# bioinfo-pf-curie/mpiBWA

Hardware: AMD Instinct MI355X
Metric: Mreads/s (whole node) 2x150 bp PE vs GRCh38-size reference; SAM bit-match (higher is better)
Workload: dtype int32

## Files before the change

### include/mpibwa_amd.h

```cpp
#ifndef MPIBWA_AMD_H
#define MPIBWA_AMD_H

#include <stdint.h>
#include <stddef.h>
#include <stdio.h>

#ifdef __cplusplus
extern "C" {
#endif

#define MEM_F_PE             0x2
#define MEM_F_NOPAIRING      0x4
#define MEM_F_ALL            0x8
#define MEM_F_NO_MULTI       0x10
#define MEM_F_NO_RESCUE      0x20
#define MEM_F_REF_HDR        0x100
#define MEM_F_SOFTCLIP       0x200
#define MEM_F_SMARTPE        0x400
#define MEM_F_PRIMARY5       0x800
#define MEM_F_KEEP_SUPP_MAPQ 0x1000

typedef uint64_t bwtint_t;

typedef struct {
// ... 132 lines not shown
int mi355x_smem_batch(const mem_opt_t *opt, int n, const uint8_t *seqs, const int64_t *off,
                      int cap, uint64_t *intv_out, int *n_out, double *kernel_ms, uint64_t *algo_bytes);
int mi355x_sa_batch(int n, const uint64_t *k, uint64_t *sa_out, double *kernel_ms, uint64_t *algo_bytes);
int mi355x_sa_batch2(int n, const uint64_t *k, uint64_t *sa_out, double *kernel_ms, int dense);
double mi355x_sa_dense_info(size_t *bytes);
int mi355x_extend_batch(const mem_opt_t *opt, int n, const uint8_t *q, const int64_t *qoff,
                        const uint8_t *t, const int64_t *toff, const int *w, const int *h0,
                        const int *end_bonus, int *out6, double *kernel_ms, uint64_t *cells);
int mi355x_extend_batch2(const mem_opt_t *opt, int n, const uint8_t *q, const int64_t *qoff,
                         const uint8_t *t, const int64_t *toff, const int *w, const int *h0,
                         const int *end_bonus, const int *early, const int *clip, int *out6,
                         uint64_t *cells, double *kernel_ms);

int64_t mi355x_chain_batch(const mem_opt_t *opt, const bntseq_t *bns, int n_reads, const int *lens, const int *l_rep,
                           const int64_t *seed_off, const uint64_t *rbeg, const int32_t *qbeg_len, int which,
                           int64_t *out, int64_t out_cap, int64_t *out_off);

int64_t mi355x_c2a_batch(const mem_opt_t *opt, const bntseq_t *bns, int n_reads, const uint8_t *reads, const int64_t *off,
                         const int *n_chains, const int *chain_rid, const float *chain_frac, const int *chain_nseeds,
                         const int64_t *seed_rbeg, const int *seed_qbeg, const int *seed_len, const int *seed_score,
                         int heavy_t, int early, int layout, int64_t *out, int64_t out_cap, int64_t *out_off,
                         uint64_t *stat4, int *n_units);

int mi355x_global_batch(const mem_opt_t *opt, int64_t l_pac, const uint8_t *pac, int n_reads, const uint8_t *reads,
                        const int64_t *off, int n_req, const int64_t *rb, const int64_t *re, const int *read,
                        const int *qb, const int *qe, const int *w, const int *truesc, int which,
                        int *out_hdr5, uint32_t *cigar_out, int cigar_cap, char *md_out, int md_cap, double *kernel_ms);
void mi355x_global_batch_counts(uint64_t out[4]);

int mi355x_pair_maxreg(void);
int mi355x_pair_batch(const mem_opt_t *opt, const bntseq_t *bns, const mem_pestat_t pes[4], int64_t n_processed, int n_pairs,
                      const void *regs, const int *n_regs, int max_len, uint8_t *status, void *desc, void *req);

int mi355x_pair_wave_maxreg(void);
int mi355x_pair_wave_batch(const mem_opt_t *opt, const bntseq_t *bns, const uint8_t *pac, const mem_pestat_t pes[4], int64_t n_processed,
                           int n_pairs, const uint8_t *reads, const int64_t *off, const void *regs, const int *reg_off, uint8_t *status,
                           void *desc, void *req, int *n_align);

int mi355x_pair_wave_xa_cap(void);
int mi355x_pair_wave_xa_batch(const mem_opt_t *opt, const bntseq_t *bns, const uint8_t *pac, const mem_pestat_t pes[4], int64_t n_processed,
                              int n_pairs, const uint8_t *reads, const int64_t *off, const void *regs, const int *reg_off, uint8_t *status,
                              void *desc, void *req, int *n_align, void *xa_req, uint8_t *xa_cnt);

int mi355x_pair_wave_lines_batch(const mem_opt_t *opt, const bntseq_t *bns, const uint8_t *pac, const mem_pestat_t pes[4], int64_t n_processed,
                                 int n_pairs, const uint8_t *reads, const int64_t *off, const void *regs, const int *reg_off, uint8_t *status,
                                 void *desc, void *req, int *n_align, void *xa_req, uint8_t *xa_cnt, uint8_t *n_lines, void *line_desc,
// ... 118 lines not shown
```

### mpibwa_amd/api.py

```python
import ctypes as C
import os

import numpy as np

from . import abi

HERE = os.path.dirname(os.path.abspath(__file__))
_LIB = None

libc = C.CDLL(None if os.environ.get("MPIBWA_SANITIZER_LIB") else "libc.so.6")
libc.free.argtypes = [C.c_void_p]

EXPORTS = [
    "mem_process_seqs", "mem_opt_init", "bwa_fill_scmat", "bwa_idx_load_from_disk", "bwa_mem2idx", "bwa_idx_destroy",
    "mi355x_index_upload", "mi355x_index_alloc", "mi355x_index_buffers", "mi355x_index_d2d", "mi355x_index_commit",
    "mi355x_finalize", "mi355x_index_build", "mi355x_index_build_gpu",
    "mi355x_smem_batch", "mi355x_sa_batch", "mi355x_sa_batch2", "mi355x_sa_dense_info", "mi355x_extend_batch", "mi355x_extend_batch2", "mi355x_matesw_batch", "mi355x_matesw_batch_counts", "mi355x_chain_batch", "mi355x_c2a_batch", "mi355x_pair_batch", "mi355x_pair_maxreg", "mi355x_fastq_scan", "mi355x_fastq_chunks", "mi355x_fastq_fill", "mi355x_last_stats", "mi355x_host_cpus", "mi355x_collect_sam", "mi355x_collect_sam_into", "mi355x_host_ksw_align2",
    "bwa_set_rg", "bwa_insert_header", "bwa_idx2mem", "mi355x_write_map", "mi355x_init", "mi355x_rank_host_threads", "mi355x_index_checksums", "mi355x_init_bcast_seconds", "mi355x_global_batch", "mi355x_global_batch_counts", "mi355x_device_count", "mi355x_device_cus", "mi355x_device_memory", "mi355x_buffer_growths", "mi355x_prewarm", "mi355x_max_calls",
    "mi355x_sam_batch", "mi355x_sam_arena_bytes", "mi355x_se_batch", "mi355x_sam_se_batch", "mi355x_seed_batch", "mi355x_pair_wave_batch", "mi355x_pair_wave_maxreg",
    "mi355x_pair_wave_xa_batch", "mi355x_pair_wave_xa_cap", "mi355x_dedup_batch", "mi355x_dedup_maxreg", "mi355x_se_wave_batch",
    "mi355x_se_lines_cap", "mi355x_se_wave_lines_batch", "mi355x_sam_se_lines_batch", "mi355x_sam_lines_row", "mi355x_sam_lines_sa_stage",
    "mi355x_pair_wave_lines_batch", "mi355x_sam_pe_lines_batch",
]


class mi355x_comm_t(C.Structure):
    BCAST = C.CFUNCTYPE(None, C.c_void_p, C.c_size_t, C.c_int, C.c_void_p)
    _fields_ = [("rank", C.c_int), ("size", C.c_int), ("bcast", BCAST), ("user", C.c_void_p)]



def load_library(build_if_missing=True):
    global _LIB
    if _LIB is not None:
        return _LIB
    path = os.path.join(HERE, "libmpibwa_amd.so")
    host_only = os.environ.get("MPIBWA_SANITIZER_LIB")
    if host_only:
        path = host_only
    if not os.path.exists(path):
        if not build_if_missing or host_only:
            raise RuntimeError("%s is missing: run python -m mpibwa_amd.build" % path)
        from .build import build
        build()
    lib = C.CDLL(path)
# ... 10 lines not shown
        fn.argtypes = argtypes

    sig("mem_opt_init", P(abi.mem_opt_t), [])
    sig("bwa_idx_load_from_disk", P(abi.bwaidx_t), [C.c_char_p, C.c_int])
    sig("mi355x_index_build", C.c_int, [C.c_char_p, C.c_char_p])
    sig("mi355x_index_build_gpu", C.c_int, [C.c_int, C.c_void_p, C.c_int64, C.c_char_p, P(C.c_double)])
    sig("mem_process_seqs", None, [P(abi.mem_opt_t), P(abi.bwt_t), P(abi.bntseq_t), P(C.c_uint8), C.c_int64, C.c_int,
                                   P(abi.bseq1_t), P(abi.mem_pestat_t)])
    sig("mi355x_index_upload", C.c_int, [C.c_int, P(abi.bwt_t), P(abi.bntseq_t), P(C.c_uint8)])
    sig("mi355x_index_alloc", C.c_int, [C.c_int, P(abi.bwt_t), P(abi.bntseq_t)])
    sig("mi355x_index_buffers", C.c_int, [P(C.c_void_p), P(C.c_size_t)] * 3)
    sig("mi355x_index_d2d", C.c_int, [C.c_int, C.c_void_p, C.c_size_t, C.c_int])
    sig("mi355x_index_commit", C.c_int, [])
    sig("mi355x_smem_batch", C.c_int, [P(abi.mem_opt_t), C.c_int, C.c_void_p, C.c_void_p, C.c_int, C.c_void_p,
                                       C.c_void_p, P(C.c_double), P(C.c_uint64)])
    sig("mi355x_sa_batch", C.c_int, [C.c_int, C.c_void_p, C.c_void_p, P(C.c_double), P(C.c_uint64)])
    sig("mi355x_sa_batch2", C.c_int, [C.c_int, C.c_void_p, C.c_void_p, P(C.c_double), C.c_int])
    sig("mi355x_sa_dense_info", C.c_double, [P(C.c_size_t)])
    sig("mi355x_extend_batch", C.c_int, [P(abi.mem_opt_t), C.c_int] + [C.c_void_p] * 8 + [P(C.c_double), P(C.c_uint64)])
    sig("mi355x_extend_batch2", C.c_int, [P(abi.mem_opt_t), C.c_int] + [C.c_void_p] * 11 + [P(C.c_double)])
    sig("mi355x_chain_batch", C.c_int64, [P(abi.mem_opt_t), C.c_void_p, C.c_int] + [C.c_void_p] * 5 + [C.c_int, C.c_void_p, C.c_int64, C.c_void_p])
    sig("mi355x_c2a_batch", C.c_int64, [P(abi.mem_opt_t), C.c_void_p, C.c_int] + [C.c_void_p] * 10 + [C.c_int] * 3 +
        [C.c_void_p, C.c_int64, C.c_void_p, C.c_void_p, C.c_void_p])
    sig("mi355x_fastq_scan", C.c_int64, [C.c_void_p, C.c_int64, C.c_int64, C.c_void_p, C.c_void_p])
    sig("mi355x_fastq_chunks", C.c_int64, [C.c_void_p, C.c_void_p, C.c_int64, C.c_int64, C.c_int64, C.c_void_p])
    sig("mi355x_fastq_fill", C.c_int64, [C.c_void_p, C.c_void_p, C.c_void_p, C.c_void_p, C.c_int64, C.c_int64, C.c_int, C.c_int, C.c_void_p])
    sig("mi355x_matesw_batch", C.c_int, [P(abi.mem_opt_t), C.c_int64, C.c_void_p, C.c_int, C.c_void_p, C.c_void_p, C.c_int] + [C.c_void_p] * 5 + [P(C.c_double)])
    sig("mi355x_last_stats", None, [P(abi.mi355x_stats_t)])
    sig("mi355x_finalize", None, [])
    sig("mi355x_host_ksw_align2", None, [C.c_int, C.c_void_p, C.c_int, C.c_void_p, C.c_void_p] + [C.c_int] * 6 + [C.c_void_p])
    sig("mi355x_host_cpus", C.c_int, [])
    sig("mi355x_host_sort_dedup_patch", C.c_int, [P(abi.mem_opt_t), P(abi.bntseq_t), C.c_void_p, C.c_void_p, C.c_void_p, C.c_int])
    sig("mi355x_host_reg2sam_se", None, [P(abi.mem_opt_t), P(abi.bntseq_t), C.c_void_p, P(abi.bseq1_t), C.c_void_p, C.c_int, C.c_int64])
    sig("mi355x_host_pestat", None, [P(abi.mem_opt_t), C.c_int64, C.c_int, C.c_void_p, C.c_void_p, C.c_void_p, C.c_int])
    sig("mi355x_host_flt_chained_seeds", None, [P(abi.mem_opt_t), P(abi.bntseq_t), C.c_void_p, C.c_int, C.c_void_p, C.c_int, C.c_void_p, C.c_void_p])
    sig("mi355x_host_sam_pe", C.c_int, [P(abi.mem_opt_t), P(abi.bntseq_t), C.c_void_p, C.c_void_p, C.c_uint64, P(abi.bseq1_t), C.c_void_p, C.c_int, C.c_void_p, C.c_int])
    sig("mi355x_collect_sam", C.c_void_p, [P(abi.bseq1_t), C.c_int, P(C.c_size_t)])
    sig("mi355x_fixmate_pair", C.c_int, [P(abi.bseq1_t), P(abi.bseq1_t), P(abi.bntseq_t)])
    sig("mi355x_fixmate", C.c_int64, [P(abi.bseq1_t), C.c_int, P(abi.bntseq_t)])
    sig("mi355x_bgzf_bound", C.c_size_t, [C.c_size_t])
    sig("mi355x_bgzf_compress", C.c_size_t, [C.c_char_p, C.c_size_t, C.c_int, C.c_void_p, C.c_size_t])
    sig("mi355x_bgzf_eof", C.c_size_t, [C.c_void_p])
    sig("mi355x_bgzf_compress_dev", C.c_size_t, [C.c_char_p, C.c_size_t, C.c_void_p, C.c_size_t])
    sig("mi355x_bgzf_dev_counts", None, [P(C.c_uint64)])
    sig("mi355x_bgzf_find_block", C.c_int64, [C.c_char_p, C.c_int64, C.c_int])
    sig("mi355x_bgzf_scan", C.c_int64, [C.c_char_p, C.c_int64, C.c_int64, P(C.c_int64), P(C.c_int64)])
# ... 242 lines not shown
        rid = np.array([c[0] for c in ch] or [0], dtype=np.int32)
        frac = np.array([c[1] for c in ch] or [0], dtype=np.float32)
        nsd = np.array([len(c[2]) for c in ch] or [0], dtype=np.int32)
        sd = np.array([s for c in ch for s in c[2]] or [(0, 0, 0, 0)], dtype=np.int64).reshape(-1, 4)
        rbeg = np.ascontiguousarray(sd[:, 0])
        qbeg, ln, sc = (np.ascontiguousarray(sd[:, k], dtype=np.int32) for k in (1, 2, 3))
        cap = n + 11 * max(int(nsd.sum()), 1) + 64
        out = np.zeros(cap, dtype=np.int64)
        out_off = np.zeros(n + 1, dtype=np.int64)
        stat = np.zeros(4, dtype=np.uint64)
        units = C.c_int(0)
        rc = self.lib.mi355x_c2a_batch(opt, C.cast(self.bns, C.c_void_p), n, flat.ctypes.data, off.ctypes.data, n_chains.ctypes.data, rid.ctypes.data,
                                       frac.ctypes.data, nsd.ctypes.data, rbeg.ctypes.data, qbeg.ctypes.data, ln.ctypes.data, sc.ctypes.data,
                                       int(heavy_t), int(early), int(layout), out.ctypes.data, cap, out_off.ctypes.data, stat.ctypes.data, C.addressof(units))
        assert rc >= 0
        res = []
        for r in range(n):
            p = int(out_off[r])
            m = int(out[p])
            res.append(out[p + 1:p + 1 + 11 * m].reshape(m, 11).copy())
        st = dict(zip(("cells", "n_ext", "n_closed", "n_diff"), (int(x) for x in stat)))
        return res, st, units.value

    REG_DT = np.dtype([("rb", "<i8"), ("re", "<i8"), ("qb", "<i4"), ("qe", "<i4"), ("rid", "<i4"), ("score", "<i4"), ("truesc", "<i4"), ("w", "<i4"),
                       ("seedcov", "<i4"), ("seedlen0", "<i4"), ("frac_rep", "<f4"), ("pad", "<i4")])
    DESC_DT = np.dtype([("rb", "<i8"), ("re", "<i8"), ("qb", "<i4"), ("qe", "<i4"), ("req", "<i4"), ("rid", "<i4"), ("flag", "<i4"), ("mapq", "<i4"),
                        ("score", "<i4"), ("sub", "<i4")])
    AREQ_DT = np.dtype([("rb", "<i8"), ("re", "<i8"), ("read", "<i4"), ("qb", "<i4"), ("qe", "<i4"), ("w2", "<i4"), ("truesc", "<i4"), ("pad", "<i4")])

    def pairs(self, opt, pes, regs, n_regs, max_len=150, n_processed=0):
        regs = np.ascontiguousarray(regs, dtype=self.REG_DT)
        assert regs.shape[1] == self.lib.mi355x_pair_maxreg()
        n_regs = np.ascontiguousarray(n_regs, dtype=np.int32)
        n_pairs = len(n_regs) // 2
        status = np.zeros(n_pairs, dtype=np.uint8)
        desc = np.zeros(2 * n_pairs, dtype=self.DESC_DT)
        req = np.zeros(2 * n_pairs, dtype=self.AREQ_DT)
        rc = self.lib.mi355x_pair_batch(opt, C.cast(self.bns, C.c_void_p), C.cast(pes, C.c_void_p), n_processed, n_pairs, regs.ctypes.data, n_regs.ctypes.data,
                                        max_len, status.ctypes.data, desc.ctypes.data, req.ctypes.data)
        if rc != 0:
            raise RuntimeError("mi355x_pair_batch: the kernel cannot use these insert-size statistics")
        return status, desc, req

    PW_DECIDED_XA = 16

    def pairs_wave_xa(self, opt, pes, reads, regs, n_processed=0):
# ... 336 lines not shown
```

### mpibwa_amd/csrc/c2a_groups.hip

```cpp
#include <hip/hip_runtime.h>
#include <hipcub/hipcub.hpp>
#include "hip_util.h"
#include "device.h"

namespace mbw {

namespace {

typedef unsigned long long u64;
typedef long long i64;
#define POS_BITS 36
#define POS_MASK ((1ull << POS_BITS) - 1)

__global__ void __launch_bounds__(64) grp_keys_kernel(int n_heavy, const int *__restrict__ hoff, const int *__restrict__ heavy, const int *__restrict__ chain_beg,
                                                      const DevChain *__restrict__ chains, u64 *__restrict__ key, int *__restrict__ val)
{
	const int h = blockIdx.x;
	if (h >= n_heavy) return;
	const int e0 = hoff[h], n = hoff[h + 1] - e0, c0 = chain_beg[heavy[h]];
	for (int t = threadIdx.x; t < n; t += 64) {
		key[e0 + t] = (u64)h << POS_BITS | (u64)chains[c0 + t].rmax0;
		val[e0 + t] = c0 + t;
	}
}
__global__ void grp_ends_kernel(int n_el, const u64 *__restrict__ key, const int *__restrict__ val, const DevChain *__restrict__ chains, u64 *__restrict__ ends)
{
// ... 19 lines not shown
}
__global__ void grp_units_kernel(int n_el, int n_heavy, const u64 *__restrict__ key2, const int *__restrict__ slot_excl, const int *__restrict__ hoff,
                                 const int *__restrict__ heavy, const int *__restrict__ reg_beg, int *__restrict__ clist, int *__restrict__ ustart,
                                 int *__restrict__ unit_rd, int *__restrict__ unit_av, unsigned int *__restrict__ n_units)
{
	const int i = blockIdx.x * blockDim.x + threadIdx.x;
	if (i >= n_el) return;
	clist[i] = (int)(unsigned)key2[i];
	const unsigned comp = (unsigned)(key2[i] >> 32);
	if (i == 0 || (unsigned)(key2[i - 1] >> 32) != comp) {
		int lo = 0, hi = n_heavy - 1;
		while (lo < hi) {
			const int mid = (lo + hi + 1) >> 1;
			if (hoff[mid] <= i) lo = mid; else hi = mid - 1;
		}
		const int rd = heavy[lo];
		ustart[comp] = i;
		unit_rd[comp] = rd;
		unit_av[comp] = reg_beg[rd] + (slot_excl[i] - slot_excl[hoff[lo]]);
	}
	if (i == n_el - 1) { ustart[comp + 1] = n_el; *n_units = comp + 1; }
}

}

static size_t cub_tmp_bytes(int n_el)
{
	size_t a = 0, b = 0, c = 0, d = 0;
	HIP_OK(hipcub::DeviceRadixSort::SortPairs(nullptr, a, (const u64 *)nullptr, (u64 *)nullptr, (const int *)nullptr, (int *)nullptr, n_el));
	HIP_OK(hipcub::DeviceScan::InclusiveScan(nullptr, b, (const u64 *)nullptr, (u64 *)nullptr, hipcub::Max(), n_el));
	HIP_OK(hipcub::DeviceScan::InclusiveSum(nullptr, c, (const int *)nullptr, (int *)nullptr, n_el));
	HIP_OK(hipcub::DeviceScan::ExclusiveSum(nullptr, d, (const int *)nullptr, (int *)nullptr, n_el));
	size_t m = a > b ? a : b;
	m = m > c ? m : c;
	m = m > d ? m : d;
	return (m + 255) & ~(size_t)255;
}
size_t c2a_groups_scratch_bytes(int n_el)
{
	const size_t n = (size_t)n_el + 64;
	return cub_tmp_bytes(n_el) + 3 * n * 8 + 4 * n * 4 + 1024;
}

void launch_c2a_groups(void *stream, int n_el, int n_heavy, const int *d_hoff, const int *d_heavy, const int *d_chain_beg, const int *d_reg_beg,
                       const DevChain *d_chains, void *d_scratch, int *d_clist, int *d_ustart, int *d_unit_rd, int *d_unit_av, unsigned int *d_n_units)
{
	if (n_el <= 0) return;
	hipStream_t st = (hipStream_t)stream;
	const size_t n = (size_t)n_el + 64;
	size_t tmp_bytes = cub_tmp_bytes(n_el);
	uint8_t *p = (uint8_t *)d_scratch;
	void *tmp = p; p += tmp_bytes;
	u64 *key_a = (u64 *)p; p += n * 8;
	u64 *key_b = (u64 *)p; p += n * 8;
	u64 *ends = (u64 *)p; p += n * 8;
	int *val_a = (int *)p; p += n * 4;
	int *val_b = (int *)p; p += n * 4;
	int *ia = (int *)p; p += n * 4;
	int *ib = (int *)p; p += n * 4;
	const dim3 grid((n_el + 255) / 256), block(256);
	hipLaunchKernelGGL(grp_keys_kernel, dim3(n_heavy), dim3(64), 0, st, n_heavy, d_hoff, d_heavy, d_chain_beg, d_chains, key_a, val_a);
	int bits = POS_BITS;
	for (int h = n_heavy; h > 0; h >>= 1) ++bits;
	HIP_OK(hipcub::DeviceRadixSort::SortPairs(tmp, tmp_bytes, key_a, key_b, val_a, val_b, n_el, 0, bits, st));
	hipLaunchKernelGGL(grp_ends_kernel, grid, block, 0, st, n_el, key_b, val_b, d_chains, ends);
	HIP_OK(hipcub::DeviceScan::InclusiveScan(tmp, tmp_bytes, ends, key_a , hipcub::Max(), n_el, st));
	hipLaunchKernelGGL(grp_flag_kernel, grid, block, 0, st, n_el, key_b, key_a, ia);
	HIP_OK(hipcub::DeviceScan::InclusiveSum(tmp, tmp_bytes, ia, ib, n_el, st));
	hipLaunchKernelGGL(grp_keys2_kernel, grid, block, 0, st, n_el, ib, val_b, d_chains, key_a, val_a );
	int bits2 = 32;
	for (int c = n_el; c > 0; c >>= 1) ++bits2;
	HIP_OK(hipcub::DeviceRadixSort::SortPairs(tmp, tmp_bytes, key_a, key_b, val_a, val_b, n_el, 0, bits2 > 64 ? 64 : bits2, st));
	HIP_OK(hipcub::DeviceScan::ExclusiveSum(tmp, tmp_bytes, val_b, ia, n_el, st));
	hipLaunchKernelGGL(grp_units_kernel, grid, block, 0, st, n_el, n_heavy, key_b, ia, d_hoff, d_heavy, d_reg_beg, d_clist, d_ustart, d_unit_rd, d_unit_av, d_n_units);
	HIP_OK(hipGetLastError());
}

C2aUnits c2a_prepare_units(void *stream, C2aGroupBufs &B, int heavy_t, int n, const int *chain_cnt, size_t n_chain_slots, const int *d_chain_beg,
                           const int *d_reg_beg, const DevChain *d_chains, int *d_nregs, void (*wait)(void *stream))
{
	C2aUnits units;
	if (heavy_t <= 0) return units;
	hipStream_t st = (hipStream_t)stream;
	int n_heavy = 0;
	int64_t n_el = 0;
	for (int i = 0; i < n; ++i)
		if (chain_cnt[i] > heavy_t) { ++n_heavy; n_el += chain_cnt[i]; }
	if (n_heavy == 0 || n_el >= 0x7fffffff) return units;
	int *hv = (int *)B.h_heavy.ensure((size_t)n_heavy * 4 + 64), *ho = (int *)B.h_hoff.ensure((size_t)(n_heavy + 1) * 4 + 64);
	int k = 0, tot = 0;
	for (int i = 0; i < n; ++i)
		if (chain_cnt[i] > heavy_t) { hv[k] = i; ho[k] = tot; tot += chain_cnt[i]; ++k; }
	ho[k] = tot;
	int *d_hv = (int *)B.heavy.ensure((size_t)n_heavy * 4), *d_ho = (int *)B.hoff.ensure((size_t)(n_heavy + 1) * 4);
	void *d_gs = B.scratch.ensure(c2a_groups_scratch_bytes((int)n_el));
	int *d_clist = (int *)B.clist.ensure((size_t)n_el * 4), *d_ustart = (int *)B.ustart.ensure((size_t)(n_el + 1) * 4);
	int *d_urd = (int *)B.unit_rd.ensure((size_t)n_el * 4), *d_uav = (int *)B.unit_av.ensure((size_t)n_el * 4);
	unsigned int *d_nu = (unsigned int *)B.nunits.ensure(64);
	units.c_rabs = (int *)B.c_rabs.ensure(n_chain_slots * 4);
	units.c_rcnt = (int *)B.c_rcnt.ensure(n_chain_slots * 4);
	HIP_OK(hipMemcpyAsync(d_hv, hv, (size_t)n_heavy * 4, hipMemcpyHostToDevice, st));
	HIP_OK(hipMemcpyAsync(d_ho, ho, (size_t)(n_heavy + 1) * 4, hipMemcpyHostToDevice, st));
	launch_c2a_groups(st, (int)n_el, n_heavy, d_ho, d_hv, d_chain_beg, d_reg_beg, d_chains, d_gs, d_clist, d_ustart, d_urd, d_uav, d_nu);
	unsigned int *nu = (unsigned int *)B.h_nunits.ensure(64);
	HIP_OK(hipMemcpyAsync(nu, d_nu, 4, hipMemcpyDeviceToHost, st));
	if (wait) wait(st);
	else HIP_OK(hipStreamSynchronize(st));
	HIP_OK(hipGetLastError());
	units.max_units = (int)nu[0]; units.heavy_t = heavy_t; units.n_units = d_nu; units.ustart = d_ustart;
	units.unit_rd = d_urd; units.unit_av = d_uav; units.clist = d_clist;
	HIP_OK(hipMemsetAsync(d_nregs, 0, (size_t)(n + 1) * 4, st));
	return units;
}

}
```

### mpibwa_amd/csrc/device.h

```cpp
#ifndef MBW_DEVICE_H
#define MBW_DEVICE_H
#include "internal.h"
#include <mutex>
#include <vector>

namespace mbw {

struct FmDev {
	const void *blk;
	const void *occ32;
	const void *occ_sb;
	const uint64_t *sa;
	const uint64_t *sa_full;
	uint64_t primary, seq_len;
	uint64_t L2[5];
	int sa_shift;
	const void *p3tab;
	int p3_k;
	const void *kmt;
	int kmt_k;
};

struct DevIndex {
	int device = -1;
// ... 81 lines not shown
};
struct DevReg {
	int64_t rb, re;
	int32_t qb, qe, rid, score, truesc, w, seedcov, seedlen0;
	float frac_rep;
	int32_t pad;
};
struct C2aParams {
	int64_t l_pac;
	int a, w, pen_clip5, pen_clip3;
	int early;
};
struct C2aUnits {
	int max_units = 0, heavy_t = 0;
	const unsigned int *n_units = nullptr;
	const int *ustart = nullptr;
	const int *unit_rd = nullptr, *unit_av = nullptr;
	const int *clist = nullptr;
	int *c_rabs = nullptr, *c_rcnt = nullptr;
};
struct C2aGroupBufs {
	PinBuf h_heavy, h_hoff, h_nunits;
	DevBuf heavy, hoff, scratch, clist, ustart, unit_rd, unit_av, nunits, c_rabs, c_rcnt;
	void release()
	{
		for (PinBuf *b : {&h_heavy, &h_hoff, &h_nunits}) b->release();
		for (DevBuf *b : {&heavy, &hoff, &scratch, &clist, &ustart, &unit_rd, &unit_av, &nunits, &c_rabs, &c_rcnt}) b->release();
	}
};
C2aUnits c2a_prepare_units(void *stream, C2aGroupBufs &B, int heavy_t, int n, const int *chain_cnt, size_t n_chain_slots, const int *d_chain_beg,
                           const int *d_reg_beg, const DevChain *d_chains, int *d_nregs, void (*wait)(void *stream) = nullptr);
void c2a_launch_order(int n, const int *nseeds, int *order);
void c2a_length_tables(const mem_opt_t *opt, int max_len, std::vector<int> &tab);
void c2a_params(const mem_opt_t *opt, int64_t l_pac, int early, C2aParams &cp, ExtParams &ep);
size_t c2a_groups_scratch_bytes(int n_el);
void launch_c2a_groups(void *stream, int n_el, int n_heavy, const int *d_hoff, const int *d_heavy, const int *d_chain_beg, const int *d_reg_beg,
                       const DevChain *d_chains, void *d_scratch, int *d_clist, int *d_ustart, int *d_unit_rd, int *d_unit_av, unsigned int *d_n_units);
#define C2A_STAT_SLOTS 256
void launch_c2a(void *stream, const C2aParams &P, const ExtParams &ep, int n_reads, const uint8_t *d_seq, const int64_t *d_off,
                const int *d_len, const int *d_chain_beg, const int *d_chain_cnt, const DevChain *d_chains, const DevSeed *d_seeds, unsigned int *d_srt,
                const int *d_reg_beg, DevReg *d_regs, int *d_nregs, const int *d_tab, int tab_stride, const uint8_t *d_pac, unsigned long long *d_counters,
                int max_len, const int *d_order = nullptr, const C2aUnits *units = nullptr );

struct ChainParams {
	int64_t l_pac;
	int w, max_chain_gap, min_chain_weight, min_seed_len, max_chain_extend;
	float mask_level, drop_ratio;
};
ChainParams chain_params(const mem_opt_t *opt, int64_t l_pac);
void contig_table(const bntseq_t *bns, std::vector<int64_t> &ann_off, std::vector<uint8_t> &ann_alt);
void launch_chain(void *stream, const ChainParams &P, int n_reads, const int *d_len, const int *d_nseeds, const int *d_lrep,
                  const int64_t *d_seed_off, const uint64_t *d_sa, const int32_t *d_qbl, const int64_t *d_ann_off, const uint8_t *d_ann_alt,
                  int n_seqs, const int *d_tab, int tab_stride, DevChain *d_chains, DevSeed *d_seeds, unsigned int *d_srt, int *d_nchains,
                  void *d_scratch);
size_t chain_scratch_bytes(int n_reads);

size_t reg_pack_tmp_bytes(int n_reads);
void launch_reg_pack(void *stream, int n_reads, const int *d_reg_beg, const int *d_nregs, int *d_reg_pos, const DevReg *d_regs, DevReg *d_packed,
                     void *d_tmp, size_t tmp_bytes, const C2aUnits *units = nullptr, const int *d_chain_beg = nullptr, const int *d_chain_cnt = nullptr);
struct C2aJob {
// ... 252 lines not shown
```

### mpibwa_amd/csrc/phase1.hip

```cpp
#include "pipeline.h"

namespace mbw {

static int c2a_early_mode() { const char *e = getenv("MPIBWA_C2A_EARLY"); return e ? atoi(e) : 1; }
static bool dev_dedup_on()
{
	const char *on = getenv("MPIBWA_DEV_DEDUP"), *off = getenv("MPIBWA_HOST_DEDUP");
	return on && atoi(on) != 0 && !(off && atoi(off) != 0);
}
static int c2a_heavy_t() { static const int t = getenv("MPIBWA_C2A_HEAVY") ? atoi(getenv("MPIBWA_C2A_HEAVY")) : 8; return t; }
static bool take_turns() { static const bool on = !(getenv("MPIBWA_TURNS") && atoi(getenv("MPIBWA_TURNS")) == 0); return on; }
static TurnLock g_smem_turn, g_c2a_turn;
static std::mutex g_pes_lock;

struct SeedTurn {
	int n_sb, cap, max_len, n_quads; size_t per_quad; bool count_blocks;
	const uint8_t *d_seq; const int64_t *d_off; const int *d_len;
	uint64_t *d_intv; int *d_nintv, *d_nseeds, *d_lrep; unsigned long long *d_cnt; void *d_scr;
	unsigned long long *cnt; int *nseeds, *lrep, *nintv;
};
static void seed_turn(hipStream_t lst, const FmDev &fm, const mem_opt_t *opt, const SeedTurn &T, EvTimer &ev_smem)
{
	stage(20);
	std::unique_lock<TurnLock> turn(g_smem_turn, std::defer_lock);
// ... 334 lines not shown
	T.d_nfirst = d_pr_first ? d_pr_nfirst + lo : nullptr;
	const bool dev_dedup = dev_dedup_on();
	EvTimer ev_ext;
	std::unique_ptr<EvTimer> ev_dd;
	if (dev_dedup) {
		ev_dd.reset(new EvTimer());
		T.ev_dd = ev_dd.get();
		T.dd = dedup_params(opt, bns->l_pac);
		T.d_dd_status = (uint8_t *)L.dd_status.ensure((size_t)n_sb);
		T.d_dd_m = (int *)L.dd_m.ensure((size_t)n_sb * 4);
		T.d_dd_keep = (int *)L.dd_keep.ensure((size_t)n_slots * 4);
		T.d_dd_list = (int *)L.dd_list.ensure(dedup_list_ints(n_sb) * 4);
		T.h_dd_status = (uint8_t *)L.h_dd_status.ensure((size_t)n_sb + 8);
		T.h_dd_m = (int *)L.h_dd_m.ensure((size_t)n_sb * 4 + 8);
		T.h_dd_keep = (int *)L.h_dd_keep.ensure((size_t)guess * 4 + 8);
	}
	extend_turn(lst, opt, bns->l_pac, T, ev_ext);
	ps.k_ext = ev_ext.ms();
	unsigned long long cnt[4] = {0, 0, 0, 0};
	for (int k = 0; k < 4; ++k)
		for (int sl = 0; sl < C2A_STAT_SLOTS; ++sl) cnt[k] += T.stat_h[sl * 8 + k];
	ps.cells = cnt[0]; ps.n_ext = cnt[1];
	if (T.early == 2 && cnt[3]) die("c2a_kernel: %llu of %llu extensions change when their row loops stop early", cnt[3], cnt[1]);
	if (cpusec_on()) fprintf(stderr, "[c2a] %llu extensions, %llu without DP, %llu cells, kernel %.2f ms\n", cnt[1], cnt[2], cnt[0], ps.k_ext);
	for (int i = 0; i < n_sb; ++i) B.reg_pos[i + 1] = B.reg_pos[i] + B.nregs[i];
	const int64_t NR = B.reg_pos[n_sb];
	B.hregs = T.hregs;
	if (NR > guess) {
		B.hregs = (DevReg *)L.h_regs2.ensure((size_t)NR * sizeof(DevReg) + 8);
		HIP_OK(hipMemcpyAsync(B.hregs, J.d_packed, (size_t)NR * sizeof(DevReg), hipMemcpyDeviceToHost, lst));
		if (dev_dedup) {
			T.h_dd_keep = (int *)L.h_dd_keep2.ensure((size_t)NR * 4 + 8);
			HIP_OK(hipMemcpyAsync(T.h_dd_keep, T.d_dd_keep, (size_t)NR * 4, hipMemcpyDeviceToHost, lst));
		}
		stream_wait(lst);
	}
	if (dev_dedup) {
		B.dd_status = T.h_dd_status; B.dd_m = T.h_dd_m; B.dd_keep = T.h_dd_keep;
		ps.k_dedup = ev_dd->ms();
		if (cpusec_on()) {
			unsigned long long c[5] = {0, 0, 0, 0, 0};
			for (int i = 0; i < n_sb; ++i) ++c[B.dd_status[i] < 5 ? B.dd_status[i] : 0];
			fprintf(stderr, "[dedup] kernels %.2f ms; reads taken %llu, more than %d regions %llu, to patch %llu\n", ps.k_dedup, c[DD_TAKEN], DD_MAXREG,
			        c[DD_HOST_MAXREG], c[DD_HOST_PATCH]);
		}
	}
}
// ... 106 lines not shown
```

### mpibwa_amd/csrc/stage_entries.hip

```cpp
#include <algorithm>
#include <atomic>
#include <cstdlib>
#include <cstring>
#include <vector>
#include "hip_util.h"
#include "device.h"
#include "host.h"

using namespace mbw;

static void need_index()
{
	if (!dev_index().ready) die("index not resident on the device: call mi355x_index_upload() first");
}

static void require_any_device()
{
	int nd = 0;
	if (hipGetDeviceCount(&nd) != hipSuccess || nd == 0) die("no HIP device visible (no CPU fallback)");
}

struct PackedReads {
	std::vector<int> lens;
	std::vector<int64_t> slot;
// ... 812 lines not shown
	d_packed.download((void *)regs.data(), (size_t)reg_pos[n_reads] * sizeof(DevReg));
	for (int k = 0; k < 4; ++k) {
		uint64_t t = 0;
		for (int sl = 0; sl < C2A_STAT_SLOTS; ++sl) t += stat[(size_t)sl * 8 + k];
		if (stat4) stat4[k] = t;
	}
	int64_t at = 0;
	for (int i = 0; i < n_reads; ++i) {
		out_off[i] = at;
		if (at + 1 + 11 * (int64_t)nregs[i] > out_cap) return -1;
		out[at++] = nregs[i];
		for (int k = 0; k < nregs[i]; ++k) {
			const DevReg &a = regs[reg_pos[i] + k];
			uint32_t fb;
			memcpy(&fb, &a.frac_rep, 4);
			const int64_t v[11] = {a.rb, a.re, a.qb, a.qe, a.rid, a.score, a.truesc, a.w, a.seedcov, a.seedlen0, (int64_t)fb};
			for (int f = 0; f < 11; ++f) out[at++] = v[f];
		}
	}
	out_off[n_reads] = at;
	return at;
}

static std::atomic<uint64_t> g_aln_counts[4];
extern "C" void mi355x_global_batch_counts(uint64_t out[4])
{
	for (int k = 0; k < 4; ++k) out[k] = g_aln_counts[k].load();
}
extern "C" int mi355x_global_batch(const mem_opt_t *opt, int64_t l_pac, const uint8_t *pac, int n_reads, const uint8_t *reads,
                                   const int64_t *off, int n_req, const int64_t *rb, const int64_t *re, const int *read,
                                   const int *qb, const int *qe, const int *w, const int *truesc, int which,
                                   int *out_hdr5, uint32_t *cigar_out, int cigar_cap, char *md_out, int md_cap, double *kernel_ms)
{
	require_any_device();
	if (n_req <= 0) return 0;
	hipStream_t st = 0;
	const PackedReads R = pack_reads(n_reads, reads, off, 4);
	const int max_len = R.max_len;
	std::vector<AlnReq> rq(n_req);
	for (int i = 0; i < n_req; ++i) {
		if (read[i] != -1 && (read[i] < 0 || read[i] >= n_reads || rb[i] < 0 || re[i] > 2 * l_pac)) die("mi355x_global_batch: bad request %d", i);
		rq[i].rb = rb[i]; rq[i].re = re[i]; rq[i].read = read[i]; rq[i].qb = qb[i]; rq[i].qe = qe[i]; rq[i].w2 = w[i]; rq[i].truesc = truesc[i];
		rq[i].pad = 0;
	}
	std::vector<int> gaptab;
	cigar_gap_table(opt, max_len, gaptab);
// ... 234 lines not shown
```

Measured before the change: 7.958.

## Group heavy-read chains per read in LDS instead of device-wide CUB sort

Replaces the device-wide radix-sort/scan grouping of chains into overlap units for heavy reads with a per-read kernel. Each read is processed by one block that sorts and scans in shared memory with a bitonic sort, and blocks are bucketed into four size classes by chain count. A small scan over per-read component counts then scatters the units into place. The aim is to cut the global sort passes and memory traffic of the old path. The cost is extra host-side ordering and a fallback to the old path when a read has more than 4096 chains. A test entry point and a debug log line are added as well.

Result: no change. 8.027 (median of 5 runs) (+0.9%).

```diff
diff --git a/include/mpibwa_amd.h b/include/mpibwa_amd.h
--- a/include/mpibwa_amd.h
+++ b/include/mpibwa_amd.h
@@ -178,6 +178,10 @@
                          int heavy_t, int early, int layout, int64_t *out, int64_t out_cap, int64_t *out_off,
                          uint64_t *stat4, int *n_units);
 
+int mi355x_c2a_groups_batch(int n_heavy, const int *hoff, const int *heavy, int n_reads, const int *chain_beg, const int *reg_beg,
+                            int n_chains, const int64_t *rmax0, const int64_t *rmax1, const int *n_seeds, int mode, int *clist,
+                            int *ustart, int *unit_rd, int *unit_av, int *path, double *kernel_ms);
+
 int mi355x_global_batch(const mem_opt_t *opt, int64_t l_pac, const uint8_t *pac, int n_reads, const uint8_t *reads,
                         const int64_t *off, int n_req, const int64_t *rb, const int64_t *re, const int *read,
                         const int *qb, const int *qe, const int *w, const int *truesc, int which,
diff --git a/mpibwa_amd/api.py b/mpibwa_amd/api.py
--- a/mpibwa_amd/api.py
+++ b/mpibwa_amd/api.py
@@ -20,7 +20,7 @@
     "mi355x_sam_batch", "mi355x_sam_arena_bytes", "mi355x_se_batch", "mi355x_sam_se_batch", "mi355x_seed_batch", "mi355x_pair_wave_batch", "mi355x_pair_wave_maxreg",
     "mi355x_pair_wave_xa_batch", "mi355x_pair_wave_xa_cap", "mi355x_dedup_batch", "mi355x_dedup_maxreg", "mi355x_se_wave_batch",
     "mi355x_se_lines_cap", "mi355x_se_wave_lines_batch", "mi355x_sam_se_lines_batch", "mi355x_sam_lines_row", "mi355x_sam_lines_sa_stage",
-    "mi355x_pair_wave_lines_batch", "mi355x_sam_pe_lines_batch",
+    "mi355x_pair_wave_lines_batch", "mi355x_sam_pe_lines_batch", "mi355x_c2a_groups_batch",
 ]
 
 
@@ -77,6 +77,8 @@
     sig("mi355x_chain_batch", C.c_int64, [P(abi.mem_opt_t), C.c_void_p, C.c_int] + [C.c_void_p] * 5 + [C.c_int, C.c_void_p, C.c_int64, C.c_void_p])
     sig("mi355x_c2a_batch", C.c_int64, [P(abi.mem_opt_t), C.c_void_p, C.c_int] + [C.c_void_p] * 10 + [C.c_int] * 3 +
         [C.c_void_p, C.c_int64, C.c_void_p, C.c_void_p, C.c_void_p])
+    sig("mi355x_c2a_groups_batch", C.c_int, [C.c_int, C.c_void_p, C.c_void_p, C.c_int, C.c_void_p, C.c_void_p, C.c_int] + [C.c_void_p] * 3 + [C.c_int] +
+        [C.c_void_p] * 5 + [P(C.c_double)])
     sig("mi355x_fastq_scan", C.c_int64, [C.c_void_p, C.c_int64, C.c_int64, C.c_void_p, C.c_void_p])
     sig("mi355x_fastq_chunks", C.c_int64, [C.c_void_p, C.c_void_p, C.c_int64, C.c_int64, C.c_int64, C.c_void_p])
     sig("mi355x_fastq_fill", C.c_int64, [C.c_void_p, C.c_void_p, C.c_void_p, C.c_void_p, C.c_int64, C.c_int64, C.c_int, C.c_int, C.c_void_p])
@@ -365,6 +367,21 @@
         st = dict(zip(("cells", "n_ext", "n_closed", "n_diff"), (int(x) for x in stat)))
         return res, st, units.value
 
+    @staticmethod
+    def c2a_groups(hoff, heavy, chain_beg, reg_beg, rmax0, rmax1, n_seeds, mode=1):
+        hoff, heavy, chain_beg, reg_beg, n_seeds = (np.ascontiguousarray(a, dtype=np.int32) for a in (hoff, heavy, chain_beg, reg_beg, n_seeds))
+        rmax0, rmax1 = (np.ascontiguousarray(a, dtype=np.int64) for a in (rmax0, rmax1))
+        n_heavy, n_el = len(heavy), int(hoff[-1])
+        assert len(hoff) == n_heavy + 1 and len(chain_beg) == len(reg_beg) and len(rmax0) == len(rmax1) == len(n_seeds)
+        out = {k: np.zeros(n_el + (k == "ustart"), dtype=np.int32) for k in ("clist", "ustart", "unit_rd", "unit_av")}
+        path, ms = C.c_int(0), C.c_double(0)
+        out["n_units"] = load_library().mi355x_c2a_groups_batch(n_heavy, hoff.ctypes.data, heavy.ctypes.data, len(chain_beg), chain_beg.ctypes.data,
+                                                          reg_beg.ctypes.data, len(rmax0), rmax0.ctypes.data, rmax1.ctypes.data, n_seeds.ctypes.data,
+                                                          int(mode), out["clist"].ctypes.data, out["ustart"].ctypes.data, out["unit_rd"].ctypes.data,
+                                                          out["unit_av"].ctypes.data, C.addressof(path), C.byref(ms))
+        out["per_read"], out["ms"] = path.value, ms.value
+        return out
+
     REG_DT = np.dtype([("rb", "<i8"), ("re", "<i8"), ("qb", "<i4"), ("qe", "<i4"), ("rid", "<i4"), ("score", "<i4"), ("truesc", "<i4"), ("w", "<i4"),
                        ("seedcov", "<i4"), ("seedlen0", "<i4"), ("frac_rep", "<f4"), ("pad", "<i4")])
     DESC_DT = np.dtype([("rb", "<i8"), ("re", "<i8"), ("qb", "<i4"), ("qe", "<i4"), ("req", "<i4"), ("rid", "<i4"), ("flag", "<i4"), ("mapq", "<i4"),
diff --git a/mpibwa_amd/csrc/c2a_groups.hip b/mpibwa_amd/csrc/c2a_groups.hip
--- a/mpibwa_amd/csrc/c2a_groups.hip
+++ b/mpibwa_amd/csrc/c2a_groups.hip
@@ -1,7 +1,10 @@
 #include <hip/hip_runtime.h>
 #include <hipcub/hipcub.hpp>
+#include <stdlib.h>
+#include <string.h>
 #include "hip_util.h"
 #include "device.h"
+#include "c2a_seg.h"
 
 namespace mbw {
 
@@ -67,6 +70,57 @@
 	if (i == n_el - 1) { ustart[comp + 1] = n_el; *n_units = comp + 1; }
 }
 
+struct SegLanes {
+	int tid, T;
+	template <class F>
+	__device__ void each(int N, F f)
+	{
+		for (int i = tid; i < N; i += T) f(i);
+		__syncthreads();
+	}
+};
+template <int P, int T>
+__global__ void __launch_bounds__(T) seg_read_kernel(int n_cls, const int *__restrict__ order, const int *__restrict__ hoff, const int *__restrict__ heavy,
+                                                     const int *__restrict__ chain_beg, const int *__restrict__ reg_beg, const DevChain *__restrict__ chains,
+                                                     int *__restrict__ clist, int *__restrict__ s_ust, int *__restrict__ s_uav, int *__restrict__ ncomp)
+{
+	__shared__ u64 lds[3 * P];
+	if ((int)blockIdx.x >= n_cls) return;
+	const int h = order[blockIdx.x];
+	const int e0 = hoff[h], n = hoff[h + 1] - e0, rd = heavy[h];
+	if (n <= 0 || n > P) return;
+	const int c0 = chain_beg[rd];
+	SegLanes x = {(int)threadIdx.x, T};
+	const int nc = seg::read_groups(x, n, chains + c0, c0, e0, reg_beg[rd], lds, lds + P, lds + 2 * P, clist + e0, s_ust + e0, s_uav + e0);
+	if (threadIdx.x == 0) ncomp[h] = nc;
+}
+__global__ void __launch_bounds__(256) seg_units_kernel(int n_heavy, int n_el, const int *__restrict__ hoff, const int *__restrict__ heavy,
+                                                        const int *__restrict__ ncomp, const int *__restrict__ base, const int *__restrict__ s_ust,
+                                                        const int *__restrict__ s_uav, int *__restrict__ ustart, int *__restrict__ unit_rd,
+                                                        int *__restrict__ unit_av, unsigned int *__restrict__ n_units)
+{
+	const int h = blockIdx.x * 4 + (threadIdx.x >> 6), lane = threadIdx.x & 63;
+	if (h >= n_heavy) return;
+	const int e0 = hoff[h], nc = ncomp[h], b = base[h], rd = heavy[h];
+	if (b < 0 || nc < 0 || nc > hoff[h + 1] - e0 || b + nc > n_el) return;
+	for (int c = lane; c < nc; c += 64) {
+		ustart[b + c] = s_ust[e0 + c];
+		unit_rd[b + c] = rd;
+		unit_av[b + c] = s_uav[e0 + c];
+	}
+	if (h == n_heavy - 1 && lane == 0) { ustart[b + nc] = n_el; *n_units = (unsigned int)(b + nc); }
+}
+
+template <int C>
+void launch_seg_class(hipStream_t st, const C2aSegPlan &plan, const int *d_hoff, const int *d_heavy, const int *d_chain_beg, const int *d_reg_beg,
+                      const DevChain *d_chains, int *d_clist, int *s_ust, int *s_uav, int *ncomp)
+{
+	const int n_cls = plan.cls_beg[C + 1] - plan.cls_beg[C];
+	if (n_cls <= 0) return;
+	hipLaunchKernelGGL((seg_read_kernel<seg::class_chains(C), seg::class_threads(C)>), dim3(n_cls), dim3(seg::class_threads(C)), 0, st, n_cls,
+	                   plan.d_order + plan.cls_beg[C], d_hoff, d_heavy, d_chain_beg, d_reg_beg, d_chains, d_clist, s_ust, s_uav, ncomp);
+}
+
 }
 
 static size_t cub_tmp_bytes(int n_el)
@@ -87,11 +141,52 @@
 	return cub_tmp_bytes(n_el) + 3 * n * 8 + 4 * n * 4 + 1024;
 }
 
-void launch_c2a_groups(void *stream, int n_el, int n_heavy, const int *d_hoff, const int *d_heavy, const int *d_chain_beg, const int *d_reg_beg,
-                       const DevChain *d_chains, void *d_scratch, int *d_clist, int *d_ustart, int *d_unit_rd, int *d_unit_av, unsigned int *d_n_units)
-{
-	if (n_el <= 0) return;
+bool c2a_groups_plan(int n_heavy, const int *h_hoff, int *h_order, const int *d_order, C2aSegPlan &plan)
+{
+	static const bool cub = [] { const char *e = getenv("MPIBWA_C2A_GROUPS"); return e && !strcmp(e, "cub"); }();
+	static_assert(sizeof plan.cls_beg / sizeof plan.cls_beg[0] == seg::N_CLASS + 1, "C2aSegPlan::cls_beg");
+	plan = C2aSegPlan();
+	if (cub || !seg::plan_order(n_heavy, h_hoff, h_order, plan.cls_beg)) return false;
+	plan.d_order = d_order;
+	return true;
+}
+
+static void launch_c2a_groups_seg(hipStream_t st, const C2aSegPlan &plan, int n_el, int n_heavy, const int *d_hoff, const int *d_heavy,
+                                  const int *d_chain_beg, const int *d_reg_beg, const DevChain *d_chains, void *d_scratch, int *d_clist, int *d_ustart,
+                                  int *d_unit_rd, int *d_unit_av, unsigned int *d_n_units)
+{
+	if (plan.cls_beg[seg::N_CLASS] != n_heavy) die("launch_c2a_groups: a plan of %d reads for %d", plan.cls_beg[seg::N_CLASS], n_heavy);
+	const size_t n = (size_t)n_el + 64;
+	size_t tmp_bytes = cub_tmp_bytes(n_el), need = 0;
+	uint8_t *p = (uint8_t *)d_scratch;
+	void *tmp = p; p += tmp_bytes;
+	int *ncomp = (int *)p; p += n * 4;
+	int *base = (int *)p; p += n * 4;
+	int *s_ust = (int *)p; p += n * 4;
+	int *s_uav = (int *)p; p += n * 4;
+	HIP_OK(hipcub::DeviceScan::ExclusiveSum(nullptr, need, (const int *)nullptr, (int *)nullptr, n_heavy));
+	if (need > tmp_bytes) die("launch_c2a_groups: the scan of %d counts needs %zu bytes, %zu at hand", n_heavy, need, tmp_bytes);
+	launch_seg_class<0>(st, plan, d_hoff, d_heavy, d_chain_beg, d_reg_beg, d_chains, d_clist, s_ust, s_uav, ncomp);
+	launch_seg_class<1>(st, plan, d_hoff, d_heavy, d_chain_beg, d_reg_beg, d_chains, d_clist, s_ust, s_uav, ncomp);
+	launch_seg_class<2>(st, plan, d_hoff, d_heavy, d_chain_beg, d_reg_beg, d_chains, d_clist, s_ust, s_uav, ncomp);
+	launch_seg_class<3>(st, plan, d_hoff, d_heavy, d_chain_beg, d_reg_beg, d_chains, d_clist, s_ust, s_uav, ncomp);
+	HIP_OK(hipcub::DeviceScan::ExclusiveSum(tmp, tmp_bytes, ncomp, base, n_heavy, st));
+	hipLaunchKernelGGL(seg_units_kernel, dim3((n_heavy + 3) / 4), dim3(256), 0, st, n_heavy, n_el, d_hoff, d_heavy, ncomp, base, s_ust, s_uav, d_ustart,
+	                   d_unit_rd, d_unit_av, d_n_units);
+	HIP_OK(hipGetLastError());
+}
+
+int launch_c2a_groups(void *stream, int n_el, int n_heavy, const int *d_hoff, const int *d_heavy, const int *d_chain_beg, const int *d_reg_beg,
+                      const DevChain *d_chains, void *d_scratch, int *d_clist, int *d_ustart, int *d_unit_rd, int *d_unit_av, unsigned int *d_n_units,
+                      const C2aSegPlan *plan)
+{
+	if (n_el <= 0) return 0;
 	hipStream_t st = (hipStream_t)stream;
+	if (plan && plan->d_order) {
+		launch_c2a_groups_seg(st, *plan, n_el, n_heavy, d_hoff, d_heavy, d_chain_beg, d_reg_beg, d_chains, d_scratch, d_clist, d_ustart, d_unit_rd,
+		                      d_unit_av, d_n_units);
+		return 1;
+	}
 	const size_t n = (size_t)n_el + 64;
 	size_t tmp_bytes = cub_tmp_bytes(n_el);
 	uint8_t *p = (uint8_t *)d_scratch;
@@ -119,12 +214,14 @@
 	HIP_OK(hipcub::DeviceScan::ExclusiveSum(tmp, tmp_bytes, val_b, ia, n_el, st));
 	hipLaunchKernelGGL(grp_units_kernel, grid, block, 0, st, n_el, n_heavy, key_b, ia, d_hoff, d_heavy, d_reg_beg, d_clist, d_ustart, d_unit_rd, d_unit_av, d_n_units);
 	HIP_OK(hipGetLastError());
+	return 0;
 }
 
 C2aUnits c2a_prepare_units(void *stream, C2aGroupBufs &B, int heavy_t, int n, const int *chain_cnt, size_t n_chain_slots, const int *d_chain_beg,
                            const int *d_reg_beg, const DevChain *d_chains, int *d_nregs, void (*wait)(void *stream))
 {
 	C2aUnits units;
+	B.n_heavy = B.n_el = B.n_units = B.most_chains = B.per_read = 0;
 	if (heavy_t <= 0) return units;
 	hipStream_t st = (hipStream_t)stream;
 	int n_heavy = 0;
@@ -132,26 +229,30 @@
 	for (int i = 0; i < n; ++i)
 		if (chain_cnt[i] > heavy_t) { ++n_heavy; n_el += chain_cnt[i]; }
 	if (n_heavy == 0 || n_el >= 0x7fffffff) return units;
-	int *hv = (int *)B.h_heavy.ensure((size_t)n_heavy * 4 + 64), *ho = (int *)B.h_hoff.ensure((size_t)(n_heavy + 1) * 4 + 64);
-	int k = 0, tot = 0;
+	int *hv = (int *)B.h_heavy.ensure((size_t)n_heavy * 8 + 64), *ho = (int *)B.h_hoff.ensure((size_t)(n_heavy + 1) * 4 + 64);
+	int k = 0, tot = 0, most = 0;
 	for (int i = 0; i < n; ++i)
-		if (chain_cnt[i] > heavy_t) { hv[k] = i; ho[k] = tot; tot += chain_cnt[i]; ++k; }
+		if (chain_cnt[i] > heavy_t) { hv[k] = i; ho[k] = tot; tot += chain_cnt[i]; most = std::max(most, chain_cnt[i]); ++k; }
 	ho[k] = tot;
-	int *d_hv = (int *)B.heavy.ensure((size_t)n_heavy * 4), *d_ho = (int *)B.hoff.ensure((size_t)(n_heavy + 1) * 4);
+	int *d_hv = (int *)B.heavy.ensure((size_t)n_heavy * 8), *d_ho = (int *)B.hoff.ensure((size_t)(n_heavy + 1) * 4);
+	C2aSegPlan plan;
+	const bool per_read = c2a_groups_plan(n_heavy, ho, hv + n_heavy, d_hv + n_heavy, plan);
 	void *d_gs = B.scratch.ensure(c2a_groups_scratch_bytes((int)n_el));
 	int *d_clist = (int *)B.clist.ensure((size_t)n_el * 4), *d_ustart = (int *)B.ustart.ensure((size_t)(n_el + 1) * 4);
 	int *d_urd = (int *)B.unit_rd.ensure((size_t)n_el * 4), *d_uav = (int *)B.unit_av.ensure((size_t)n_el * 4);
 	unsigned int *d_nu = (unsigned int *)B.nunits.ensure(64);
 	units.c_rabs = (int *)B.c_rabs.ensure(n_chain_slots * 4);
 	units.c_rcnt = (int *)B.c_rcnt.ensure(n_chain_slots * 4);
-	HIP_OK(hipMemcpyAsync(d_hv, hv, (size_t)n_heavy * 4, hipMemcpyHostToDevice, st));
+	HIP_OK(hipMemcpyAsync(d_hv, hv, (size_t)n_heavy * (per_read ? 8 : 4), hipMemcpyHostToDevice, st));
 	HIP_OK(hipMemcpyAsync(d_ho, ho, (size_t)(n_heavy + 1) * 4, hipMemcpyHostToDevice, st));
-	launch_c2a_groups(st, (int)n_el, n_heavy, d_ho, d_hv, d_chain_beg, d_reg_beg, d_chains, d_gs, d_clist, d_ustart, d_urd, d_uav, d_nu);
+	B.per_read = launch_c2a_groups(st, (int)n_el, n_heavy, d_ho, d_hv, d_chain_beg, d_reg_beg, d_chains, d_gs, d_clist, d_ustart, d_urd, d_uav, d_nu,
+	                               per_read ? &plan : nullptr);
 	unsigned int *nu = (unsigned int *)B.h_nunits.ensure(64);
 	HIP_OK(hipMemcpyAsync(nu, d_nu, 4, hipMemcpyDeviceToHost, st));
 	if (wait) wait(st);
 	else HIP_OK(hipStreamSynchronize(st));
 	HIP_OK(hipGetLastError());
+	B.n_heavy = n_heavy; B.n_el = (int)n_el; B.n_units = (int)nu[0]; B.most_chains = most;
 	units.max_units = (int)nu[0]; units.heavy_t = heavy_t; units.n_units = d_nu; units.ustart = d_ustart;
 	units.unit_rd = d_urd; units.unit_av = d_uav; units.clist = d_clist;
 	HIP_OK(hipMemsetAsync(d_nregs, 0, (size_t)(n + 1) * 4, st));
diff --git a/mpibwa_amd/csrc/c2a_seg.h b/mpibwa_amd/csrc/c2a_seg.h
--- /dev/null
+++ b/mpibwa_amd/csrc/c2a_seg.h
@@ -0,0 +1,99 @@
+#pragma once
+#include <stdint.h>
+
+#if defined(__HIPCC__)
+#define SEG_HD __host__ __device__
+#else
+#define SEG_HD
+#endif
+
+namespace mbw {
+namespace seg {
+
+typedef unsigned long long u64;
+enum {
+	T_BITS = 12,
+	MAX_CHAINS = 1 << T_BITS,
+	N_CLASS = 4
+};
+#define SEG_T_MASK ((u64)(mbw::seg::MAX_CHAINS - 1))
+
+SEG_HD constexpr int class_chains(int c) { return c == 0 ? 4096 : c == 1 ? 1024 : c == 2 ? 256 : 64; }
+SEG_HD constexpr int class_threads(int c) { return c == 0 ? 512 : c == 1 ? 256 : c == 2 ? 128 : 64; }
+SEG_HD constexpr int class_of(int n) { return n <= 64 ? 3 : n <= 256 ? 2 : n <= 1024 ? 1 : n <= MAX_CHAINS ? 0 : -1; }
+
+SEG_HD inline int pow2_ceil(int n)
+{
+	int p = 2;
+	while (p < n) p <<= 1;
+	return p;
+}
+
+template <class X>
+SEG_HD inline void bitonic(X &x, u64 *k, int Pn)
+{
+	for (int kk = 2; kk <= Pn; kk <<= 1)
+		for (int j = kk >> 1; j > 0; j >>= 1)
+			x.each(Pn >> 1, [&](int t) {
+				const int i = ((t & ~(j - 1)) << 1) | (t & (j - 1)), l = i | j;
+				const u64 a = k[i], b = k[l];
+				if ((a > b) == ((i & kk) == 0)) { k[i] = b; k[l] = a; }
+			});
+}
+
+template <class X, class OP>
+SEG_HD inline u64 *scan_incl(X &x, u64 *a, u64 *b, int Pn, OP op)
+{
+	for (int d = 1; d < Pn; d <<= 1) {
+		x.each(Pn, [&](int i) { b[i] = i >= d ? op(a[i - d], a[i]) : a[i]; });
+		u64 *t = a; a = b; b = t;
+	}
+	return a;
+}
+
+template <class X, class CH>
+SEG_HD inline int read_groups(X &x, int n, const CH *ch, int c0, int e0, int av0, u64 *K, u64 *A, u64 *B, int *clist, int *ust, int *uav)
+{
+	const int Pn = pow2_ceil(n);
+	x.each(Pn, [&](int i) { K[i] = i < n ? ((u64)ch[i].rmax0 << T_BITS | (u64)i) : ~0ull; });
+	bitonic(x, K, Pn);
+	x.each(Pn, [&](int i) { A[i] = i < n ? (u64)ch[(int)(K[i] & SEG_T_MASK)].rmax1 : 0; });
+	u64 *R = scan_incl(x, A, B, Pn, [](u64 p, u64 q) { return p > q ? p : q; });
+	u64 *F = R == A ? B : A;
+	x.each(Pn, [&](int i) { F[i] = i < n && (i == 0 || (K[i] >> T_BITS) >= R[i - 1]) ? 1 : 0; });
+	u64 *C = scan_incl(x, F, R, Pn, [](u64 p, u64 q) { return p + q; });
+	u64 *D = C == F ? R : F;
+	const int n_comp = (int)C[n - 1];
+	x.each(Pn, [&](int i) { D[i] = i < n ? ((C[i] - 1) << T_BITS | (K[i] & SEG_T_MASK)) : ~0ull; });
+	bitonic(x, D, Pn);
+	x.each(Pn, [&](int i) { K[i] = i < n ? (u64)(uint32_t)ch[(int)(D[i] & SEG_T_MASK)].n_seeds : 0; });
+	const u64 *S = scan_incl(x, K, C, Pn, [](u64 p, u64 q) { return p + q; });
+	x.each(n, [&](int i) {
+		const int comp = (int)(D[i] >> T_BITS);
+		clist[i] = c0 + (int)(D[i] & SEG_T_MASK);
+		if (i == 0 || (int)(D[i - 1] >> T_BITS) != comp) {
+			ust[comp] = e0 + i;
+			uav[comp] = av0 + (i ? (int)S[i - 1] : 0);
+		}
+	});
+	return n_comp;
+}
+
+inline bool plan_order(int n_heavy, const int *hoff, int *order, int cls_beg[N_CLASS + 1])
+{
+	int cnt[N_CLASS] = {0};
+	for (int h = 0; h < n_heavy; ++h) {
+		const int c = class_of(hoff[h + 1] - hoff[h]);
+		if (c < 0) return false;
+		++cnt[c];
+	}
+	cls_beg[0] = 0;
+	for (int c = 0; c < N_CLASS; ++c) cls_beg[c + 1] = cls_beg[c] + cnt[c];
+	int at[N_CLASS];
+	for (int c = 0; c < N_CLASS; ++c) at[c] = cls_beg[c];
+	for (int h = 0; h < n_heavy; ++h) order[at[class_of(hoff[h + 1] - hoff[h])]++] = h;
+	return true;
+}
+
+}
+}
diff --git a/mpibwa_amd/csrc/device.h b/mpibwa_amd/csrc/device.h
--- a/mpibwa_amd/csrc/device.h
+++ b/mpibwa_amd/csrc/device.h
@@ -127,6 +127,7 @@
 struct C2aGroupBufs {
 	PinBuf h_heavy, h_hoff, h_nunits;
 	DevBuf heavy, hoff, scratch, clist, ustart, unit_rd, unit_av, nunits, c_rabs, c_rcnt;
+	int n_heavy = 0, n_el = 0, n_units = 0, most_chains = 0, per_read = 0;
 	void release()
 	{
 		for (PinBuf *b : {&h_heavy, &h_hoff, &h_nunits}) b->release();
@@ -139,8 +140,14 @@
 void c2a_length_tables(const mem_opt_t *opt, int max_len, std::vector<int> &tab);
 void c2a_params(const mem_opt_t *opt, int64_t l_pac, int early, C2aParams &cp, ExtParams &ep);
 size_t c2a_groups_scratch_bytes(int n_el);
-void launch_c2a_groups(void *stream, int n_el, int n_heavy, const int *d_hoff, const int *d_heavy, const int *d_chain_beg, const int *d_reg_beg,
-                       const DevChain *d_chains, void *d_scratch, int *d_clist, int *d_ustart, int *d_unit_rd, int *d_unit_av, unsigned int *d_n_units);
+struct C2aSegPlan {
+	const int *d_order = nullptr;
+	int cls_beg[5] = {0, 0, 0, 0, 0};
+};
+bool c2a_groups_plan(int n_heavy, const int *h_hoff, int *h_order, const int *d_order, C2aSegPlan &plan);
+int launch_c2a_groups(void *stream, int n_el, int n_heavy, const int *d_hoff, const int *d_heavy, const int *d_chain_beg, const int *d_reg_beg,
+                      const DevChain *d_chains, void *d_scratch, int *d_clist, int *d_ustart, int *d_unit_rd, int *d_unit_av, unsigned int *d_n_units,
+                      const C2aSegPlan *plan = nullptr);
 #define C2A_STAT_SLOTS 256
 void launch_c2a(void *stream, const C2aParams &P, const ExtParams &ep, int n_reads, const uint8_t *d_seq, const int64_t *d_off,
                 const int *d_len, const int *d_chain_beg, const int *d_chain_cnt, const DevChain *d_chains, const DevSeed *d_seeds, unsigned int *d_srt,
diff --git a/mpibwa_amd/csrc/phase1.hip b/mpibwa_amd/csrc/phase1.hip
--- a/mpibwa_amd/csrc/phase1.hip
+++ b/mpibwa_amd/csrc/phase1.hip
@@ -380,7 +380,9 @@
 		for (int sl = 0; sl < C2A_STAT_SLOTS; ++sl) cnt[k] += T.stat_h[sl * 8 + k];
 	ps.cells = cnt[0]; ps.n_ext = cnt[1];
 	if (T.early == 2 && cnt[3]) die("c2a_kernel: %llu of %llu extensions change when their row loops stop early", cnt[3], cnt[1]);
-	if (cpusec_on()) fprintf(stderr, "[c2a] %llu extensions, %llu without DP, %llu cells, kernel %.2f ms\n", cnt[1], cnt[2], cnt[0], ps.k_ext);
+	if (cpusec_on())
+		fprintf(stderr, "[c2a] %llu extensions, %llu without DP, %llu cells, kernel %.2f ms; groups: %d heavy reads, %d chains (at most %d of a read), %d units, %s\n",
+		        cnt[1], cnt[2], cnt[0], ps.k_ext, L.grp.n_heavy, L.grp.n_el, L.grp.most_chains, L.grp.n_units, L.grp.per_read ? "per read" : "device-wide");
 	for (int i = 0; i < n_sb; ++i) B.reg_pos[i + 1] = B.reg_pos[i] + B.nregs[i];
 	const int64_t NR = B.reg_pos[n_sb];
 	B.hregs = T.hregs;
diff --git a/mpibwa_amd/csrc/stage_entries.hip b/mpibwa_amd/csrc/stage_entries.hip
--- a/mpibwa_amd/csrc/stage_entries.hip
+++ b/mpibwa_amd/csrc/stage_entries.hip
@@ -858,6 +858,55 @@
 	return at;
 }
 
+extern "C" int mi355x_c2a_groups_batch(int n_heavy, const int *hoff, const int *heavy, int n_reads, const int *chain_beg, const int *reg_beg,
+                                       int n_chains, const int64_t *rmax0, const int64_t *rmax1, const int *n_seeds, int mode, int *clist,
+                                       int *ustart, int *unit_rd, int *unit_av, int *path, double *kernel_ms)
+{
+	require_any_device();
+	if (path) *path = 0;
+	if (n_heavy <= 0) return 0;
+	if (mode != 0 && mode != 1) die("mi355x_c2a_groups_batch: mode %d", mode);
+	if (hoff[0] != 0) die("mi355x_c2a_groups_batch: hoff[0] = %d", hoff[0]);
+	for (int h = 0; h < n_heavy; ++h) {
+		const int cnt = hoff[h + 1] - hoff[h], rd = heavy[h];
+		if (cnt <= 0 || rd < 0 || rd >= n_reads || chain_beg[rd] < 0 || (int64_t)chain_beg[rd] + cnt > n_chains)
+			die("mi355x_c2a_groups_batch: heavy read %d: read %d, %d chains", h, rd, cnt);
+	}
+	const int n_el = hoff[n_heavy];
+	std::vector<DevChain> hch(std::max(n_chains, 1));
+	memset((void *)hch.data(), 0, hch.size() * sizeof(DevChain));
+	for (int c = 0; c < n_chains; ++c) {
+		if (rmax0[c] < 0 || rmax1[c] < 0 || rmax0[c] >> 36 || rmax1[c] >> 36) die("mi355x_c2a_groups_batch: chain %d: window beyond 36 bits", c);
+		hch[c].rmax0 = rmax0[c]; hch[c].rmax1 = rmax1[c]; hch[c].n_seeds = n_seeds[c];
+	}
+	hipStream_t st = 0;
+	std::vector<int> order(n_heavy);
+	DevArr<int> d_order((size_t)n_heavy * 4);
+	C2aSegPlan plan;
+	const bool per_read = mode == 1 && c2a_groups_plan(n_heavy, hoff, order.data(), d_order, plan);
+	if (per_read) HIP_OK(hipMemcpy(d_order, order.data(), (size_t)n_heavy * 4, hipMemcpyHostToDevice));
+	const size_t e4 = (size_t)n_el * 4;
+	DevArr<int> d_hoff((size_t)(n_heavy + 1) * 4, hoff), d_heavy((size_t)n_heavy * 4, heavy), d_cbeg((size_t)n_reads * 4, chain_beg),
+		d_rbeg((size_t)n_reads * 4, reg_beg), d_clist(e4), d_ustart(e4 + 4), d_urd(e4), d_uav(e4);
+	DevArr<DevChain> d_ch(hch.size() * sizeof(DevChain), hch.data());
+	DevArr<void> d_gs(c2a_groups_scratch_bytes(n_el));
+	DevArr<unsigned int> d_nu(64);
+	d_clist.fill(0xff); d_ustart.fill(0xff); d_urd.fill(0xff); d_uav.fill(0xff); d_nu.zero();
+	Timer tm;
+	tm.start(st);
+	const int ran = launch_c2a_groups(st, n_el, n_heavy, d_hoff, d_heavy, d_cbeg, d_rbeg, d_ch, d_gs, d_clist, d_ustart, d_urd, d_uav, d_nu,
+	                                  per_read ? &plan : nullptr);
+	const double ms = tm.stop(st);
+	if (kernel_ms) *kernel_ms = ms;
+	HIP_OK(hipStreamSynchronize(st));
+	HIP_OK(hipGetLastError());
+	unsigned int nu = 0;
+	d_nu.download(&nu, 4);
+	d_clist.download(clist, e4); d_ustart.download(ustart, e4 + 4); d_urd.download(unit_rd, e4); d_uav.download(unit_av, e4);
+	if (path) *path = ran;
+	return (int)nu;
+}
+
 static std::atomic<uint64_t> g_aln_counts[4];
 extern "C" void mi355x_global_batch_counts(uint64_t out[4])
 {
```
